# FireMines/zk_stark_project

Measured on AMD Instinct MI355X. Metric: STARK proofs/sec + prove-time ms, MiMC AIR 2^20-step trace, higher is better.
Workload: dtype f128 (u128 mod 2^128-45*2^40+1); 1 GPU; MiMC AIR 2^20-step trace, blowup=8 (BASELINE configs[1]); trace_length=1048576, trace_width=1, blowup=8, num_queries=40, grinding=21, fri_folding=16, fri_remainder_max_degree=7, parallelism=replicas1

## Files before the change

__graft_entry__.py:

```python
import os
import subprocess
import sys

ROOT = os.path.dirname(os.path.abspath(__file__))


def build() -> None:
    env = dict(os.environ)
    jobs = str(min(16, os.cpu_count() or 1))
    subprocess.check_call(["make", "-j", jobs, "-C", os.path.join(ROOT, "zk_stark_project_amd", "csrc")], env=env)
    subprocess.check_call(["make", "-j", jobs, "-C", os.path.join(ROOT, "oracle")], env=env)
    subprocess.check_call(["make", "-j", jobs, "-C", os.path.join(ROOT, "tests", "native")], env=env)
    subprocess.check_call(["make", "-j", jobs, "-C", os.path.join(ROOT, "tests", "native"), "-f", "deep_inv_check.mk"],
                          env=env)
    if ROOT not in sys.path:
        sys.path.insert(0, ROOT)
    import zk_stark_project_amd
    from zk_stark_project_amd import _native
    _native.load()


def smoke() -> None:
    for p in (ROOT, os.path.join(ROOT, "tests")):
        if p not in sys.path:
            sys.path.insert(0, p)
    from zk_stark_project_amd import AIR_MIMC, MimcProver, ProofOptions, _native
    from zk_stark_project_amd.field import to_bytes
    import oracle_ref

    ctx = _native.Context(0)
    opts = ProofOptions(40, 8, 12)
    prover = MimcProver(opts, ctx)
    n = 1 << 12
    trace = prover.build_trace(42 * 10**6, n)
    pub = prover.get_pub_inputs(trace).to_elements()
    proof = prover.prove(trace)
    ref, _ = oracle_ref.prove(AIR_MIMC, trace.to_bytes(), 1, n, to_bytes(pub), opts)
    assert proof.to_bytes() == ref, "GPU proof differs from the CPU oracle"
    assert oracle_ref.verify(AIR_MIMC, proof.to_bytes(), to_bytes(pub), opts) == 0, "proof rejected"
    _native.verify(AIR_MIMC, proof.to_bytes(), pub, opts)
    ctx.close()
    print(f"smoke ok: MiMC 2^12 proof, {len(proof)} bytes, bit-exact vs oracle")


if __name__ == "__main__":
    build()
# ... 3 lines not shown
```

zk_stark_project_amd/csrc/kernels.hip:

```cpp
#include "kernels_dev.hpp"

using kc::rev_bits;
using kc::static_for;

namespace {

__global__ void k_expand_powers(felt* out, uint64_t count, const felt* lo_tab, const felt* hi_tab) {
  for (uint64_t e = blockIdx.x * (uint64_t)TPB + threadIdx.x; e < count; e += (uint64_t)gridDim.x * TPB)
    out[e] = mul(lo_tab[e & 2047], hi_tab[e >> 11]);
}

__global__ void k_build_levels(felt* tab, uint32_t top) {
  const felt* topl = tab + ((1ull << top) - 1);
  uint64_t total = (1ull << top) - 1;
  for (uint64_t e = blockIdx.x * (uint64_t)TPB + threadIdx.x; e < total; e += (uint64_t)gridDim.x * TPB) {
    uint32_t t = 63 - __builtin_clzll(e + 1);
    uint64_t j = e + 1 - (1ull << t);
    tab[e] = topl[j << (top - t)];
  }
}

__global__ void k_build_coset_scale(felt* S, uint32_t logn, uint32_t B, const felt* tw, uint32_t logN,
                                    const felt* glo, const felt* ghi, felt ninv) {
  uint64_t total = (uint64_t)B << logn;
// ... 15 lines not shown
  const uint64_t pl = blockIdx.x * (uint64_t)TPB + threadIdx.x;
  if (pl >= nR) return;
  felt x[CE];
  static_for<0, CE>([&](auto uu) {
    constexpr int u = decltype(uu)::value;
    x[u] = mul(recv[blk[u] * nR + pl], Si[((uint64_t)u << logn) + p0 + pl]);
  });
  const felt* winv = consts + C;
  static_for<0, kc::ilog2_const(CE)>([&](auto ss) {
    constexpr int len = CE >> decltype(ss)::value, h = len / 2;
    static_for<0, CE / len>([&](auto bb) {
      constexpr int b0 = decltype(bb)::value * len;
      static_for<0, h>([&](auto jj) {
        constexpr int j = decltype(jj)::value;
        const felt u = x[b0 + j], v = x[b0 + j + h];
        x[b0 + j] = add(u, v);
        x[b0 + j + h] = j == 0 ? sub(u, v) : mul(sub(u, v), winv[j * (CE / len)]);
      });
    });
  });
  static_for<0, CE>([&](auto mm) {
    constexpr int m = decltype(mm)::value;
    if ((uint32_t)m < C) out[m * nR + pl] = mul(x[kc::rev_const(m, kc::ilog2_const(CE))], consts[m]);
  });
  if (hi_flag) {
    uint32_t nz = 0;
    static_for<0, CE>([&](auto mm) {
      constexpr int m = decltype(mm)::value;
      const felt v = x[kc::rev_const(m, kc::ilog2_const(CE))];
      if ((uint32_t)m >= C) nz |= (uint32_t)((v.lo | v.hi) != 0);
    });
    if (__builtin_amdgcn_ballot_w64(nz != 0) && (threadIdx.x & 63) == 0) hi_flag[0] = 1u;
  }
}

__global__ __launch_bounds__(TPB) void k_dt_eval_consts(int air, const felt* __restrict__ cc, felt k, felt wl,
                                                        const felt* __restrict__ aval, const felt* __restrict__ zinv,
                                                        uint32_t ce, uint32_t w, uint32_t num_t,
                                                        felt* __restrict__ out) {
  __shared__ felt red0[TPB], red1[TPB];
  const uint32_t t = threadIdx.x;
  if (air == ZKP_AIR_MIMC) {
    for (uint32_t u = t; u < ce; u += TPB) out[u] = mul(zinv[u], cc[0]);
    if (t == 0) {
      const felt b0 = cc[1], b1 = cc[2], c0 = mul(b0, aval[0]), c1 = mul(b1, aval[1]);
      out[ce] = add(b0, b1);
      out[ce + 1] = add(mul(b0, wl), b1);
      out[ce + 2] = add(c0, c1);
      out[ce + 3] = add(mul(c0, wl), c1);
    }
    return;
  }
  const bool gu = air == ZKP_AIR_GLOBAL_UPDATE;
  const uint32_t W = gu ? w : w / 2;
  felt s0 = zero(), s1 = zero();
  for (uint32_t c = t; c < W; c += TPB) {
    felt a = zero(), b = zero(), b0 = zero(), b1 = zero();
    if (gu) {
      const uint32_t d = W / 2;
      if (c < d) { a = mul(cc[c], k); b = neg(a); }
      else a = neg(cc[c - d]);
      b0 = cc[num_t + c];
      s0 = add(s0, mul(b0, aval[c]));
    } else {
      b0 = cc[num_t + c];
      b1 = cc[num_t + W + c];
// ... 1406 lines not shown
           hipLaunchKernelGGL(k_deep_lincomb<false>, g, dim3(TPB), 0, s, coef, w, n, p0, np, gamma, cpg, out));
    return;
  }
  LAUNCH(prof, "deep_lincomb", s, (double)(w + 1) * np * 16.0,
         hipLaunchKernelGGL(k_deep_lincomb<true>, g, dim3(TPB), 0, s, coef, w, n, p0, np, gamma, cpg, scratch));
  LAUNCH(prof, "deep_lincomb", s, (double)(G + 1) * np * 16.0,
         hipLaunchKernelGGL(k_sum_groups, dim3(blocks_for(np)), dim3(TPB), 0, s, scratch, G, np, out));
}

void launch_deep(Prof& prof, hipStream_t s, const DeepArgs& a, felt* out) {
  uint64_t N = 1ull << (a.logn + a.logBl);
  LAUNCH(prof, "deep", s, (double)N * ((a.w + a.C) * 16.0 + 32.0),
         hipLaunchKernelGGL(k_deep, dim3(blocks_for((N + EVAL_CH - 1) / EVAL_CH)), dim3(TPB), 0, s, a, a.inv, out));
}

void launch_comp_dft(Prof& prof, hipStream_t s, const felt* recv, const uint32_t* blk, const felt* Si,
                     const felt* consts, uint32_t ce, uint32_t C, uint32_t logn, uint64_t p0, uint64_t nR, felt* out,
                     uint32_t* hi_flag) {
  const double bytes = (double)nR * (2 * ce + C) * 16.0;
  const dim3 g(blocks_for(nR));
  switch (ce) {
    case 2: LAUNCH(prof, "comp_dft", s, bytes, hipLaunchKernelGGL(k_comp_dft<2>, g, dim3(TPB), 0, s, recv, blk, Si,
                                                                   consts, C, logn, p0, nR, out, hi_flag)); break;
    case 4: LAUNCH(prof, "comp_dft", s, bytes, hipLaunchKernelGGL(k_comp_dft<4>, g, dim3(TPB), 0, s, recv, blk, Si,
                                                                   consts, C, logn, p0, nR, out, hi_flag)); break;
    case 8: LAUNCH(prof, "comp_dft", s, bytes, hipLaunchKernelGGL(k_comp_dft<8>, g, dim3(TPB), 0, s, recv, blk, Si,
                                                                   consts, C, logn, p0, nR, out, hi_flag)); break;
    case 16: LAUNCH(prof, "comp_dft", s, bytes, hipLaunchKernelGGL(k_comp_dft<16>, g, dim3(TPB), 0, s, recv, blk,
                                                                    Si, consts, C, logn, p0, nR, out, hi_flag)); break;
    default: launch_fail(ZKP_ERR_UNSUPPORTED_AIR, "composition DFT supports ce in {2, 4, 8, 16}");
  }
}

void launch_gather_multi(Prof& prof, hipStream_t s, const GatherSeg* segs, uint32_t nseg, uint64_t max_count,
                         const uint64_t* idx, uint32_t* out, double bytes) {
  LAUNCH(prof, "gather", s, bytes,
         hipLaunchKernelGGL(k_gather_multi, dim3(blocks_for(max_count), nseg), dim3(TPB), 0, s, segs, idx, out));
}

void launch_gather_felts(Prof& prof, hipStream_t s, const felt* src, const uint64_t* idx, felt* out, uint64_t count) {
  LAUNCH(prof, "gather", s, count * 32.0,
         hipLaunchKernelGGL(k_gather_felts, dim3(blocks_for(count)), dim3(TPB), 0, s, src, idx, out, count));
}

void launch_gather_digests(Prof& prof, hipStream_t s, const uint32_t* nodes, const uint64_t* idx, uint32_t* out,
                           uint64_t count) {
  LAUNCH(prof, "gather", s, count * 40.0,
         hipLaunchKernelGGL(k_gather_digests, dim3(blocks_for(count)), dim3(TPB), 0, s, nodes, idx, out, count));
}

void launch_gu_trace(Prof& prof, hipStream_t s, const felt* masked, const felt* raw, const felt* local,
                     uint64_t ndev, felt kinv, uint64_t n, felt* tile_buf, felt* out) {
  const uint32_t tiles = (uint32_t)((n + GU_TILE - 1) / GU_TILE);
  LAUNCH(prof, "gu_trace_sums", s, (double)ndev * GU_D_DEV * 16.0,
         hipLaunchKernelGGL(k_gu_tile_sums, dim3(tiles, GU_D_DEV), dim3(TPB), 0, s, masked, raw, local, ndev, kinv,
                            n, tile_buf));
  LAUNCH(prof, "gu_trace_scan", s, (double)tiles * GU_D_DEV * 32.0,
         hipLaunchKernelGGL(k_gu_tile_scan, dim3(GU_D_DEV), dim3(64), 0, s, tile_buf, tiles));
  LAUNCH(prof, "gu_trace_write", s, (double)n * 2 * GU_D_DEV * 16.0 + (double)ndev * GU_D_DEV * 16.0,
         hipLaunchKernelGGL(k_gu_tile_write, dim3(tiles, 2 * GU_D_DEV), dim3(TPB), 0, s, masked, raw, local, ndev,
                            kinv, n, tile_buf, out));
}

void launch_tu_states(Prof& prof, hipStream_t s, felt* states, const felt* x, const felt* xs, const felt* y,
                      uint32_t bs, felt pr_inv, felt lr_inv, felt ac_inv) {
  LAUNCH(prof, "tu_states", s, (double)bs * (2 * TU_FE + TU_AC + TU_HALF) * 16.0,
// ... 74 lines not shown
```

zk_stark_project_amd/csrc/ntt.hip:

```cpp
#include "kernels_common.hpp"
#include "ntt_plan.hpp"

#include <mutex>

using kc::static_for;
using kc::rev_bits;

namespace {

struct NttKArgs {
  const felt* src;
  felt* dst;
  const felt* scale;
  const felt* tw;
  uint64_t src_stride, dst_stride;
  uint32_t src_div, scale_mod;
  uint32_t logn, s0, K, lo, T, Tl, logT, logTl, dit;
};

__global__ __launch_bounds__(TPB) void k_ntt_pass(NttKArgs a) {
  extern __shared__ felt lds[];
  const uint32_t bidx = blockIdx.y;
  const felt* src = a.src + (uint64_t)(bidx / a.src_div) * a.src_stride;
  felt* dst = a.dst + (uint64_t)bidx * a.dst_stride;
  const felt* scale = a.scale ? a.scale + ((uint64_t)(bidx % a.scale_mod) << a.logn) : nullptr;
  const uint32_t K = a.K, T = a.T, Tl = a.Tl, lo = a.lo;
  const uint32_t E = T << K;
  const uint64_t g0 = (uint64_t)blockIdx.x * T;
  const uint64_t hi0 = g0 >> lo;
  const uint64_t l0 = (Tl == T) ? (g0 & ((1ull << lo) - 1)) : 0;
  const uint32_t qmask = (1u << K) - 1;

  for (uint32_t e = threadIdx.x; e < E; e += TPB) {
    uint32_t ll = e & (Tl - 1);
    uint32_t rest = e >> a.logTl;
    uint32_t q = rest & qmask;
    uint32_t hl = rest >> K;
    uint64_t addr = ((hi0 + hl) << (lo + K)) + ((uint64_t)q << lo) + l0 + ll;
    felt v = src[addr];
    if (scale) v = mul(v, scale[addr]);
    lds[(q << a.logT) + (hl * Tl) + ll] = v;
  }
  __syncthreads();
  for (uint32_t ls = 0; ls < K; ls++) {
    const uint32_t s = a.s0 + ls;
    const uint32_t pbit = a.dit ? ls : (K - 1 - ls);
    const uint32_t lev = a.dit ? s : (a.logn - 1 - s);
    const felt* twl = a.tw + ((1ull << lev) - 1);
    const uint32_t pmask = (1u << pbit) - 1;
    for (uint32_t bf = threadIdx.x; bf < (E >> 1); bf += TPB) {
      uint32_t gg = bf & (T - 1);
      uint32_t qq = bf >> a.logT;
      uint32_t q = ((qq >> pbit) << (pbit + 1)) | (qq & pmask);
      uint32_t q2 = q | (1u << pbit);
      uint64_t l = l0 + (gg & (Tl - 1));
      uint64_t j = ((uint64_t)(q & pmask) << lo) | l;
      felt w = twl[j];
      uint32_t i0 = (q << a.logT) + gg, i1 = (q2 << a.logT) + gg;
      felt x = lds[i0], y = lds[i1];
      if (a.dit) {
        felt t = mul(y, w);
        lds[i0] = add(x, t);
        lds[i1] = sub(x, t);
      } else {
        lds[i0] = add(x, y);
        lds[i1] = mul(sub(x, y), w);
      }
    }
    __syncthreads();
  }
  for (uint32_t e = threadIdx.x; e < E; e += TPB) {
    uint32_t ll = e & (Tl - 1);
    uint32_t rest = e >> a.logTl;
    uint32_t q = rest & qmask;
    uint32_t hl = rest >> K;
    uint64_t addr = ((hi0 + hl) << (lo + K)) + ((uint64_t)q << lo) + l0 + ll;
    dst[addr] = lds[(q << a.logT) + (hl * Tl) + ll];
  }
}

struct Ntt8Args {
  const felt* src;
  felt* dst;
  const felt* scale;
  const felt* tw;
  uint64_t src_stride, dst_stride;
  uint32_t src_div, scale_mod;
  uint32_t logn, s0, K, lo, logT, logTl;
  uint32_t tile_major;
};

template <bool DIT>
__device__ __forceinline__ felt ntt_tw(const Ntt8Args& a, uint32_t j, uint32_t pbit) {
  uint32_t s = DIT ? a.s0 + pbit : a.s0 + a.K - 1 - pbit;
  uint32_t lev = DIT ? s : a.logn - 1 - s;
  return a.tw[((1u << lev) - 1) + j];
}

#ifdef ZKP_NTT_NOGMEM
#define NTT_LD(p) (make((uint64_t)(uintptr_t)(p), (uint64_t)threadIdx.x))
#define NTT_ST(p, v)                                               \
  do {                                                            \
    const felt v_ = (v);                                          \
    if (v_.lo == 0x123456789ull && v_.hi == 0xabcdefull) *(p) = v_; \
  } while (0)
#else
#define NTT_LD(p) (*(p))
#define NTT_ST(p, v) (*(p) = (v))
#endif

#ifdef ZKP_NTT_NOBFLY
template <bool FAST>
__device__ __forceinline__ felt bmul(felt a, felt b, Rare& q) { return make(a.lo ^ b.lo, a.hi ^ b.hi); }
template <bool FAST>
__device__ __forceinline__ felt badd(felt a, felt b, Rare& q) { return make(a.lo + b.lo, a.hi + b.hi); }
__device__ __forceinline__ felt nsub(felt a, felt b) { return make(a.lo - b.lo, a.hi - b.hi); }
#else
template <bool FAST>
__device__ __forceinline__ felt bmul(felt a, felt b, Rare& q) { return dmul<FAST>(a, b, q); }
template <bool FAST>
__device__ __forceinline__ felt badd(felt a, felt b, Rare& q) { return dadd<FAST>(a, b, q); }
__device__ __forceinline__ felt nsub(felt a, felt b) { return sub(a, b); }
// ... 54 lines not shown
  }
#else
  bfly<DIT, FAST>(x0, y0, w0, q);
  bfly<DIT, FAST>(x1, y1, w1, q);
#endif
}

template <bool DIT, int NT, int KC, bool SMALL>
__device__ __forceinline__ void ntt8_tile(const Ntt8Args& a, uint32_t bidx, uint32_t tile, felt* lds) {
  constexpr int E = NT * 8;
  constexpr uint32_t K = KC;
  constexpr uint32_t LOGNT = NT == 512 ? 9 : 8;
  constexpr uint32_t logT = LOGNT + 3 - KC;
  constexpr uint32_t T = 1u << logT;
  static_assert(T == 1 || T >= 4, "the LDS swizzles take rows of 1 or >= 4 felts");
  const uint32_t Tl = 1u << a.logTl, lo = a.lo;
  auto lidx = [](uint32_t q, uint32_t x) -> uint32_t {
    if constexpr (T == 1) {
      (void)x;
      return q ^ ((q >> 3) & 7u) ^ (((q >> 6) & 1u) << 3);
    } else if constexpr (T >= 32) {
      return q * T + (x ^ (q & 15u));
    } else if constexpr (T == 16 && DIT) {
      return q * T + (x ^ (q & 7u));
    } else if constexpr (T == 16) {
      return q * T + (x ^ ((q & 7u) | ((((q >> 2) ^ (q >> 4)) & 1u) << 3)));
    } else if constexpr (T == 8) {
      return (q ^ (((q >> 2) ^ (q >> 3)) & 1u)) * T + (x ^ (q & 7u));
    } else {
      const uint32_t b1 = (q >> 1) & 1u, b23 = ((q >> 2) ^ (q >> 3)) & 1u, b25 = ((q >> 2) ^ (q >> 5)) & 1u;
      return (q ^ (b23 | (b25 << 1))) * T + (x ^ (b1 | (b23 << 1)));
    }
  };
  const felt* src = a.src + (uint64_t)(bidx / a.src_div) * a.src_stride;
  felt* dst = a.dst + (uint64_t)bidx * a.dst_stride;
  const felt* scale = a.scale ? a.scale + ((uint64_t)(bidx % a.scale_mod) << a.logn) : nullptr;
  const uint64_t g0 = (uint64_t)tile << logT;
  const uint32_t hi0 = (uint32_t)(g0 >> lo);
  const uint32_t l0 = (Tl == T) ? (uint32_t)(g0 & ((1ull << lo) - 1)) : 0;
  const uint32_t qmask = (1u << K) - 1;
  const uint32_t tid = threadIdx.x;

  auto gaddr = [&](uint32_t gg, uint32_t q) -> uint32_t {
    uint32_t hl = gg >> a.logTl, ll = gg & (Tl - 1);
    return ((hi0 + hl) << (lo + K)) + (q << lo) + l0 + ll;
  };
  (void)qmask;
  const bool staged = a.logTl < (T >= 8 ? 3u : 2u);
  auto staged_elem = [&](uint32_t e, uint32_t& slot) -> uint32_t {
    uint32_t ll = e & (Tl - 1), rest = e >> a.logTl;
    uint32_t q = rest & ((1u << K) - 1), hl = rest >> K;
    slot = lidx(q, hl * Tl + ll);
    return ((hi0 + hl) << (lo + K)) + (q << lo) + l0 + ll;
  };
  if (staged) {
    auto stage_in = [&](auto fast_c, Rare& q) {
      constexpr bool FAST = decltype(fast_c)::value;
#pragma unroll
      for (int i = 0; i < 8; i++) {
        uint32_t slot;
        uint32_t ad = staged_elem(tid + i * NT, slot);
        felt v = NTT_LD(src + ad);
        if (scale) v = bmul<FAST>(v, NTT_LD(scale + ad), q);
        lds[slot] = v;
      }
    };
    Rare q;
// ... 152 lines not shown
}

template <bool DIT, int NT, int KC, bool SMALL>
__global__ __launch_bounds__(NT, (NT == 256 && KC == 11) ? 5 : 1) void k_ntt8(Ntt8Args a) {
  extern __shared__ felt lds[];
  uint32_t bidx = blockIdx.x, tile = blockIdx.y;
  if (a.tile_major) {
    const uint32_t B = gridDim.x, i = blockIdx.y * B + blockIdx.x, k = i >> 3;
    tile = (k / B) * 8 + (i & 7);
    bidx = k % B;
  }
  ntt8_tile<DIT, NT, KC, SMALL>(a, bidx, tile, lds);
}

}

void preload_ntt_module() {
  hipFuncAttributes fa;
  (void)hipFuncGetAttributes(&fa, (const void*)k_ntt_pass);
}

static void launch_ntt_radix2(Prof& prof, hipStream_t s, const NttBatch& b, uint32_t logn, bool dit,
                              const felt* tw) {
  bool first = true;
  for (const NttPass& ps : ntt_plan(logn, dit, b.batches)) {
    NttKArgs a;
    a.src = first ? b.src : b.dst;
    a.dst = b.dst;
    a.scale = first ? b.scale : nullptr;
    a.tw = tw;
    a.src_stride = first ? b.src_stride : b.dst_stride;
    a.dst_stride = b.dst_stride;
    a.src_div = first ? b.src_div : 1;
    a.scale_mod = b.scale_mod ? b.scale_mod : 1;
    a.logn = logn;
    a.s0 = ps.s0;
    a.K = ps.K;
    a.lo = ps.lo;
    a.T = 1u << ps.logT;
    a.Tl = 1u << ps.logTl;
    a.logT = ps.logT;
    a.logTl = ps.logTl;
    a.dit = dit ? 1 : 0;
    uint64_t groups = 1ull << (logn - ps.K);
    dim3 grid((uint32_t)(groups >> ps.logT), b.batches);
    size_t shmem = (size_t)(a.T << ps.K) * sizeof(felt);
    LAUNCH(prof, dit ? "ntt_dit_r2" : "ntt_dif_r2", s, (double)b.batches * (1ull << logn) * 16.0 * (a.scale ? 3 : 2),
           hipLaunchKernelGGL(k_ntt_pass, grid, dim3(TPB), shmem, s, a));
    first = false;
  }
}

#define ZKP_NTT8_KERNELS(X)                                                                \
  X(true, 256, 6, true) X(true, 256, 8, true) X(true, 256, 11, true)                       \
  X(true, 256, 6, false) X(true, 256, 7, false) X(true, 256, 8, false)                     \
  X(true, 256, 9, false) X(true, 512, 9, false)                                            \
  X(false, 256, 6, true) X(false, 256, 7, true) X(false, 256, 8, true) X(false, 256, 11, true) \
  X(false, 256, 6, false) X(false, 256, 7, false) X(false, 256, 8, false)                  \
  X(false, 256, 9, false) X(false, 512, 9, false)

void launch_ntt(Prof& prof, hipStream_t s, const NttBatch& b, uint32_t logn, bool dit, const felt* tw,
                uint32_t logN, int only_pass) {
  if (logN > 28)
    launch_fail(ZKP_ERR_TRACE_SHAPE, "NTT domain over 2^28 points (n * blowup)");
  if (logn < 11) {
    if (only_pass <= 0) launch_ntt_radix2(prof, s, b, logn, dit, tw);
    return;
  }
  static std::mutex attr_mu;
  static uint64_t attr_devs = 0;
  int dev = 0;
  (void)hipGetDevice(&dev);
  {
  std::lock_guard<std::mutex> attr_lock(attr_mu);
  if (!(attr_devs >> (dev & 63) & 1)) {
#define X(D, NT, KK, S) \
  (void)hipFuncSetAttribute((const void*)k_ntt8<D, NT, KK, S>, hipFuncAttributeMaxDynamicSharedMemorySize, NT * 8 * 16);
    ZKP_NTT8_KERNELS(X)
#undef X
    attr_devs |= 1ull << (dev & 63);
  }
  }
  const NttPlan plan = ntt_plan(logn, dit, b.batches);
  for (uint32_t p = 0; p < plan.n; p++) {
    const NttPass& ps = plan.pass[p];
    if (only_pass >= 0 && (uint32_t)only_pass != p) continue;
    Ntt8Args a;
    bool first = p == 0;
    a.src = first ? b.src : b.dst;
    a.dst = b.dst;
    a.scale = first ? b.scale : nullptr;
    a.tw = tw;
    a.src_stride = first ? b.src_stride : b.dst_stride;
    a.dst_stride = b.dst_stride;
    a.src_div = first ? b.src_div : 1;
    a.scale_mod = b.scale_mod ? b.scale_mod : 1;
    a.logn = logn;
    a.s0 = ps.s0;
    a.K = ps.K;
    a.lo = ps.lo;
    a.logT = ps.logT;
    a.logTl = ps.logTl;
    uint64_t groups = 1ull << (logn - ps.K);
    dim3 grid(b.batches, (uint32_t)(groups >> a.logT));
    a.tile_major = first && b.src_div > 1 && grid.y % 8 == 0;
    size_t shmem = (size_t)(1u << ps.K) * (1u << a.logT) * sizeof(felt);
    const double arr = (double)(1ull << logn) * 16.0;
    const uint32_t src_arrays = first ? (b.batches + a.src_div - 1) / a.src_div : b.batches;
    const uint32_t scale_rows = a.scale ? (a.scale_mod < b.batches ? a.scale_mod : b.batches) : 0;
    const double bytes = arr * ((double)src_arrays + scale_rows + b.batches);
    const uint32_t nt = 1u << ps.lognt;
#define X(D, NT, KK, S)                                                              \
  if (dit == D && nt == NT && ps.K == KK && ps.small == S)                           \
    LAUNCH(prof, D ? "ntt_dit" : "ntt_dif", s, bytes,                                \
           hipLaunchKernelGGL((k_ntt8<D, NT, KK, S>), grid, dim3(NT), shmem, s, a)); \
  else
    ZKP_NTT8_KERNELS(X)
    launch_fail(ZKP_ERR_DEVICE, "internal: NTT pass of an unplanned size");
#undef X
  }
}
```

zk_stark_project_amd/csrc/ntt_plan.hpp:

```cpp
#pragma once
#include <stdint.h>

struct NttPass {
  uint32_t s0, K, lo;
  uint32_t lognt;
  uint32_t logT, logTl;
  bool small;
};

struct NttPlan {
  uint32_t n = 0;
  NttPass pass[4];
  const NttPass* begin() const { return pass; }
  const NttPass* end() const { return pass + n; }
};

inline uint32_t ntt_split_stages(uint32_t stages, uint32_t Ks[4]) {
  const uint32_t KMAX = 8;
  const uint32_t npass = (stages + KMAX - 1) / KMAX;
  uint32_t rem = stages;
  for (uint32_t p = 0; p < npass; p++) {
    const uint32_t left = npass - p;
    uint32_t k = (rem + left - 1) / left;
    if (left > 1) {
      const uint32_t k3 = k / 3 * 3;
      if (k3 >= 3 && rem - k3 <= KMAX * (left - 1)) k = k3;
    }
    Ks[p] = k;
    rem -= k;
  }
  return npass;
}

inline NttPlan ntt_plan(uint32_t logn, bool dit, uint32_t batches) {
  NttPlan pl;
  if (logn == 0 || logn > 32) return pl;
  const bool radix2 = logn < 11;
  uint32_t Ks[4] = {0, 0, 0, 0};
  if (logn == 11) {
    pl.n = 1;
    Ks[0] = 11;
  } else if (logn >= 17 && logn <= 20) {
    pl.n = 2;
    Ks[0] = dit ? 11 : logn - 11;
    Ks[1] = dit ? logn - 11 : 11;
  } else {
    pl.n = ntt_split_stages(logn, Ks);
  }
  uint32_t s0 = 0;
  for (uint32_t p = 0; p < pl.n; s0 += Ks[p], p++) {
    NttPass& ps = pl.pass[p];
    ps.s0 = s0;
    ps.K = Ks[p];
    ps.lo = dit ? s0 : logn - s0 - ps.K;
    ps.small = ps.lo == 0;
    ps.lognt = !radix2 && ps.K == 9 && batches >= 8 ? 9 : 8;
    const uint32_t loge = radix2 ? 12 : ps.lognt + 3, logG = logn - ps.K;
    ps.logT = loge - ps.K < logG ? loge - ps.K : logG;
    ps.logTl = ps.logT < ps.lo ? ps.logT : ps.lo;
  }
  return pl;
}
```

zk_stark_project_amd/csrc/prover.cpp:

```cpp
#include "prover_internal.hpp"

#include <mutex>

using namespace zkpi;

namespace zkpi {

int ProofRun::init(int air_id, const felt* d_trace_in, uint32_t width, uint64_t n_rows, const zkp_felt* pub_elems,
                   uint64_t n_pub, uint8_t** proof, uint64_t* proof_len) {
  d_trace = d_trace_in;
  w = width;
  n = n_rows;
  int rc = check_options(o);
  if (rc) return rc;
  if (n < 8 || (n & (n - 1)) || w == 0 || w > 255) return ZKP_ERR_TRACE_SHAPE;
  if (!proof || !proof_len || (n_pub && !pub_elems)) return ZKP_ERR_ARGUMENT;
  B = o->blowup_factor; F = o->fri_folding_factor;
  logn = ilog2(n); logB = ilog2(B); logN = logn + logB;
  N = 1ull << logN;
  if (logN > MAX_LOG_DOMAIN || logn > MAX_LOG_TRACE) return ZKP_ERR_TRACE_SHAPE;
  rc = check_fri_shape(n, o);
  if (rc) return rc;
  R = (uint32_t)cm->world; rank = (uint32_t)cm->rank;
  if (R == 0 || (R & (R - 1)) || R > B || rank >= R) return ZKP_ERR_ARGUMENT;
// ... 98 lines not shown
    }
    const bool mimc_check = air.id == ZKP_AIR_MIMC && w == 1 && R == 1 && lastcol_shape();
    const bool piped = h_trace && grp.size() > 1;
    const size_t G = grp.size();
    if (piped) {
      ctx->events(G + 2);
      HIP_CHECK(hipEventRecord(ctx->ev_fork, st));
      HIP_CHECK(hipStreamWaitEvent(ctx->side, ctx->ev_fork, 0));
    }
    if (late_pairs) {
      if (!piped) throw ZkpFail{ZKP_ERR_DEVICE, "paired host trace without column groups"};
      HIP_CHECK(hipMemcpy2DAsync(const_cast<felt*>(d_trace) + (size_t)d * n, n * 16, h_trace + (size_t)d * n, n * 16,
                                 16, d, hipMemcpyHostToDevice, ctx->side));
      HIP_CHECK(hipEventRecord(ctx->up_ev[G], ctx->side));
    }
    for (uint32_t g = 0; g < grp.size(); g++) {
      const uint32_t c0 = grp[g].first, cw = grp[g].second;
      felt* dcol = const_cast<felt*>(d_trace) + (size_t)c0 * n;
      if (piped) {
        HIP_CHECK(hipMemcpyAsync(dcol, h_trace + (size_t)c0 * n, (size_t)cw * n * 16, hipMemcpyHostToDevice,
                                 ctx->side));
        HIP_CHECK(hipEventRecord(ctx->up_ev[g], ctx->side));
        HIP_CHECK(hipStreamWaitEvent(st, ctx->up_ev[g], 0));
      } else if (h_trace && g == 0) {
        ctx->upload(dcol, h_trace, (size_t)w * n * 16);
      }
      if (g == 0 && mimc_check) {
        uint32_t* dflag = ctx->buf<uint32_t>("mimc_bad", 4);
        HIP_CHECK(hipEventRecord(ctx->ev_fork, st));
        HIP_CHECK(hipStreamWaitEvent(ctx->side, ctx->ev_fork, 0));
        HIP_CHECK(hipMemsetAsync(dflag, 0, 16, ctx->side));
        launch_mimc_check(pf, ctx->side, d_trace, n, air.a_val[0], air.a_val[1], dflag);
        early_check_launch(dflag, ctx->side);
      }
      if (c0 >= wd && early_pairs) HIP_CHECK(hipStreamWaitEvent(st, ctx->ev_check, 0));
      if (c0 >= wd && early_pairs && early_check_failed()) {
        paired = false;
        gu_lazy_on = false;
      } else if (c0 >= wd) {
        const uint32_t i0 = c0 - d;
        if (!early_pairs) launch_gu_check(pf, st, d_trace, d, logn, air.k, i0, cw, 0, logn, gu_cval, gu_bad);
        launch_gu_coef(pf, st, coef, d, logn, air.k, ctx->itws(logN) + ((n >> 1) - 1), i0, cw, 0, n, gu_cval);
        if (!gu_lazy_on) launch_gu_lde(pf, st, tlde, d, logn, logBl, air.k, i0, cw, gu_cval, l0_table());
        continue;
      }
      NttBatch ib{dcol, coef + (size_t)c0 * n, nullptr, n, n, 1, 1, cw};
      launch_ntt(pf, st, ib, logn, false, ctx->itws(logN), logN);
      NttBatch lb{coef + (size_t)c0 * n, tlde + (size_t)c0 * Bl * n, Sj0, n, n, Bl, Bl, cw * Bl};
      launch_ntt(pf, st, lb, logn, true, ctx->tws(logN), logN);
    }
    if (late_pairs) {
      HIP_CHECK(hipStreamWaitEvent(st, ctx->up_ev[G], 0));
      launch_gu_check(pf, st, d_trace, d, logn, air.k, 0, d, 0, 0, gu_cval, gu_bad);
      launch_gu_coef(pf, st, coef, d, logn, air.k, ctx->itws(logN) + ((n >> 1) - 1), 0, d, 0, n, gu_cval);
      if (!gu_lazy_on) launch_gu_lde(pf, st, tlde, d, logn, logBl, air.k, 0, d, gu_cval, l0_table());
      HIP_CHECK(hipEventRecord(ctx->up_ev[G + 1], ctx->side));
      HIP_CHECK(hipStreamWaitEvent(ctx->copy, ctx->up_ev[G + 1], 0));
      late_h_trace = h_trace;
    }
  }
  {
    MerkleTail draw{};
    draw.op = MERKLE_TAIL_DRAW_COEFFS;
    draw.coin_seed = dt_seed;
    draw.method = o->batching_constraints;
    draw.ncoef = ncoef;
// ... 9 lines not shown
    }
  }
  troot_d = R > 1 ? ttree.top_d + 8 : ttree.nodes + 8;
  if (!coeffs_drawn && !host_channel)
    launch_dt_draw_coeffs(pf, st, dt_seed, troot_d, o->batching_constraints, ncoef, dt_cc);
  ctx->stage_end("1_trace_commit");
}

void ProofRun::constraint_stage() {
  eval_stage();
  composition_stage();
}

void ProofRun::eval_stage() {
  comp = ctx->buf<felt>("comp", (size_t)(cel ? cel : 1) * n);
  constraint_eval(ctx, air, logn, logB, logce, u0, cel, j0, logBl, cx, twn, dt_cc, dt_aval, tlde, comp, coef, cm);
}

bool ProofRun::lastcol_shape() const {
  static const bool no_derive = getenv("ZKP_NO_DERIVE_LAST") != nullptr;
  return allow_shortcuts && !no_derive && logce == logB && C >= 2 && C <= 8 && cel == Bl && u0 == j0;
}

void ProofRun::composition_stage() {
  comp = ctx->buf<felt>("comp", (size_t)(cel ? cel : 1) * n);
  acoef = coef + (size_t)w * n;
  clde = ctx->buf<felt>("clde", (size_t)C * Bl * n);
  bool z_drawn = false;
  wn_root = root_of_unity(logn);
  {
    const uint64_t nR = n >> logR, p0 = (uint64_t)rank * nR;
    const bool derive = lastcol_shape() && !(pre_checked && early_check_failed());
    derive_last = derive;
    if (derive) {
      lc_bad = ctx->buf<uint32_t>("lc_bad", 4);
      HIP_CHECK(hipMemsetAsync(lc_bad, 0, 16, st));
    }
    felt* cint = derive ? ctx->buf<felt>("comp_int", (size_t)(cel ? cel : 1) * n) : comp;
    if (cel) {
      NttBatch ib{comp, cint, nullptr, n, n, 1, 1, cel};
      launch_ntt(pf, st, ib, logn, false, ctx->itws(logN), logN);
    }
    felt* recv = cint;
    if (R > 1) recv = composition_exchange(cint, nR);
    const std::string dkey = "comp_dft_" + std::to_string(logn) + "_" + std::to_string(logce) + "_" +
                             std::to_string(C) + "_" + std::to_string(R) + "_" + std::to_string(celmax);
    felt* dcoefs = ctx->buf<felt>(dkey + "_coefs", (size_t)C + ce / 2);
    uint32_t* dblk = ctx->buf<uint32_t>(dkey + "_blk", ce);
    if (!ctx->have_cached(dkey)) {
      const std::vector<felt> dc = comp_dft_consts(n, logce, C);
      std::vector<uint32_t> blk(ce);
      for (uint32_t u = 0; u < ce; u++) {
        uint32_t s = ce_owner(u);
        blk[u] = s * celmax + (u - ce_first(s));
      }
      ctx->upload(dcoefs, dc.data(), dc.size() * 16);
      ctx->upload(dblk, blk.data(), blk.size() * 4);
    }
    felt* slice = R > 1 ? ctx->buf<felt>("comp_ag_send", (size_t)C * nR) : acoef;
    launch_comp_dft(pf, st, recv, dblk, ctx->Si(logn, logB, logce), dcoefs, ce, C, logn, p0, nR, slice,
                    derive ? lc_bad : nullptr);
    if (R > 1 && derive) {
      lc_flags = ctx->buf<uint32_t>("lc_flags", 4 * (size_t)R);
      cm->all_gather(st, lc_bad, lc_flags, 16);
    }
    if (R > 1) {
      composition_gather_lde(slice, derive, nR, p0);
    } else {
      NttBatch lb{acoef, clde, Sj0, n, n, Bl, Bl, (derive ? C - 1 : C) * Bl};
      launch_ntt(pf, st, lb, logn, true, ctx->tws(logN), logN);
    }
    LastCol lc{};
    if (derive) lc = LastCol{comp, last_col_kappa(ctx, logn, logB, C) + 2 * (size_t)j0, clde + (size_t)(C - 1) * Bl * n};
    MerkleTail draw{};
    draw.op = MERKLE_TAIL_DRAW_Z;
    draw.coin_seed = dt_seed;
    draw.wn = wn_root;
    draw.logn = logn;
    draw.out = dt_zz;
    draw.pw = dt_pw;
    z_drawn = commit_rows(ctx, cm, 0, clde, n, C, logB, logn, R > 1, "ctree", ctree, T.constraint_root,
                          host_channel, host_channel ? nullptr : &draw, derive ? &lc : nullptr);
  }
  croot_d = R > 1 ? ctree.top_d + 8 : ctree.nodes + 8;
  if (!z_drawn && !host_channel) launch_dt_draw_z(pf, st, dt_seed, croot_d, wn_root, logn, dt_zz, dt_pw);
  ctx->stage_end("2_constraints_commit");
}

void ProofRun::ood_values() {
  const uint64_t cnt = (uint64_t)Bl * n;
  deep_inv = ctx->buf<felt>("deep_inv", cnt);
  felt* scratch = ctx->buf<felt>("deep_inv_scratch", deep_den_scratch(cnt));
  const PointMap pm{cx + j0, twn, logn};
  const PointMap pm8{coset_points8(ctx, logn, logB) + j0,
// ... 369 lines not shown
  if (!late_h_trace) return;
  const uint32_t d = w / 2;
  HIP_CHECK(hipMemcpyAsync(const_cast<felt*>(d_trace) + (size_t)d * n, late_h_trace + (size_t)d * n,
                           (size_t)d * n * 16, hipMemcpyHostToDevice, ctx->copy));
  launch_gu_check(pf, ctx->copy, d_trace, d, logn, air.k, 0, d, 0, logn, nullptr, gu_bad);
  late_h_trace = nullptr;
  gu_late_check = true;
}

void ProofRun::early_check_launch(uint32_t* dflag, hipStream_t s) {
  HIP_CHECK(hipMemcpyAsync(ctx->host_flag(), dflag, 4, hipMemcpyDeviceToHost, s));
  HIP_CHECK(hipEventRecord(ctx->ev_check, s));
  pre_checked = true;
}

bool ProofRun::early_check_failed() {
  if (!pre_checked) return false;
  HIP_CHECK(hipEventSynchronize(ctx->ev_check));
  return *ctx->host_flag() != 0;
}

bool ProofRun::pair_failed() {
  if (!paired) return false;
  late_pairs_upload();
  if (gu_late_check) HIP_CHECK(hipStreamSynchronize(ctx->copy));
  std::vector<uint32_t> f(gu_flags ? 4 * (size_t)R : 4);
  ctx->download(f.data(), gu_flags ? gu_flags : gu_bad, f.size() * 4);
  for (uint32_t v : f)
    if (v) return true;
  return false;
}

bool ProofRun::lastcol_failed() {
  if (!derive_last) return false;
  std::vector<uint32_t> f(lc_flags ? 4 * (size_t)R : 4);
  ctx->download(f.data(), lc_flags ? lc_flags : lc_bad, f.size() * 4);
  for (uint32_t v : f)
    if (v) return true;
  return false;
}

int prove_impl(zkp_ctx* ctx, zkp_comm* cm, int air_id, const felt* d_trace, uint32_t w, uint64_t n,
               const zkp_felt* pub_elems, uint64_t n_pub, const zkp_proof_options* o, uint8_t** proof,
               uint64_t* proof_len, zkp_transcript* tr_out, const zkp_felt* h_trace) {
  for (int attempt = 0;; attempt++) {
    ProofRun run(ctx, cm, o);
    run.allow_shortcuts = attempt == 0;
    int rc = run.init(air_id, d_trace, w, n, pub_elems, n_pub, proof, proof_len);
    if (rc) return rc;
    run.setup();
    run.trace_stage(h_trace);
    run.constraint_stage();
    run.ood_stage();
    run.deep_stage();
    run.fri_stage();
    run.grind_stage();
    if (run.pair_failed() || run.lastcol_failed()) {
      if (!run.h_partial) h_trace = nullptr;
      continue;
    }
    return run.finish(proof, proof_len, tr_out);
  }
}

void drain_streams(zkp_ctx* ctx) {
  (void)hipStreamSynchronize(ctx->copy);
  (void)hipStreamSynchronize(ctx->side);
// ... 89 lines not shown
```

zk_stark_project_amd/csrc/prover_internal.hpp:

```cpp
#pragma once
#include <algorithm>
#include <array>
#include <chrono>
#include <cstdio>
#include <cstdlib>
#include <cstring>
#include <map>
#include <memory>
#include <stdexcept>
#include <string>
#include <utility>
#include <vector>

#include "../../include/zkp.h"
#include "blake3.hpp"
#include "comm.hpp"
#include "zkp_internal.hpp"

using namespace fp;

#include "host_stark.hpp"

using namespace zkh;

// ... 431 lines not shown
  std::vector<FriLayer> layers;
  std::vector<felt> remainder;
  bool dev_tail = false;
  bool dev_query = false;
  FullGatherArgs ga{};
  uint64_t* dpos = nullptr;
  const uint32_t* full_d = nullptr;
  std::vector<uint32_t> full_h;
  std::vector<uint64_t> raw_pos;
  felt* rem_d = nullptr;
  uint32_t* rcommit_d = nullptr;
  unsigned long long* dres = nullptr;
  unsigned long long dnonce = ~0ull;
  static constexpr uint64_t grind_chunk = 1ull << 22;
  uint64_t nonce = 0;
  bool allow_shortcuts = true;
  bool paired = false;
  felt* gu_cval = nullptr;
  uint32_t* gu_bad = nullptr;
  uint32_t* gu_flags = nullptr;
  bool gu_lazy_on = false;
  bool gu_late_check = false;
  const zkp_felt* late_h_trace = nullptr;
  void late_pairs_upload();
  GuLazy gu_lazy{};
  const felt* l0_table();
  bool pair_failed();
  bool derive_last = false;
  bool lastcol_shape() const;
  uint32_t* lc_bad = nullptr;
  uint32_t* lc_flags = nullptr;
  bool lastcol_failed();
  bool pre_checked = false;
  void early_check_launch(uint32_t* dflag, hipStream_t s);
  bool early_check_failed();
  bool h_partial = false;
  bool host_channel = false;

  ProofRun(zkp_ctx* c, zkp_comm* m, const zkp_proof_options* opts)
      : ctx(c), cm(m), o(opts), st(c->stream), pf(c->prof) {
    memset(&T, 0, sizeof T);
  }
  uint32_t ce_owner(uint32_t u) const { return (u << cstep) / Bl; }
  uint32_t ce_first(uint32_t s) const {
    uint32_t u = 0;
    while (u < ce && ce_owner(u) < s) u++;
    return u;
  }
  int init(int air_id, const felt* d_trace_in, uint32_t width, uint64_t n_rows, const zkp_felt* pub_elems,
           uint64_t n_pub, uint8_t** proof, uint64_t* proof_len);
  void setup();
  void trace_stage(const zkp_felt* h_trace);
  void constraint_stage();
  void eval_stage();
  void composition_stage();
  void ood_values();
  void ood_stage();
  void deep_stage();
  void fri_stage();
  FriCursor fri_layers();
  void fri_round_trip(const FriCursor& c);
  void grind_stage();
  int finish(uint8_t** proof, uint64_t* proof_len, zkp_transcript* tr_out);
  void trace_column_sharded(const zkp_felt* h_trace, uint32_t cpt, uint32_t wi, uint32_t d);
  const zkp_felt* gather_host_slices(const zkp_felt* h_trace);
  felt* composition_exchange(felt* cint, uint64_t nR);
// ... 70 lines not shown
```

zk_stark_project_amd/csrc/zkp_internal.hpp:

```cpp
#pragma once
#include <hip/hip_runtime.h>
#include <stdint.h>

#include <string>
#include <vector>

#include "felt.hpp"

struct ProfRec {
  const char* name;
  double bytes;
  hipEvent_t start, stop;
};
struct Prof {
  bool enabled = false;
  std::string only;
  bool open = false;
  std::vector<ProfRec> pending;
  std::vector<hipEvent_t> pool;
  hipEvent_t get_event();
  void begin(const char* name, hipStream_t s, double bytes);
  void end(hipStream_t s);
};

[[noreturn]] void launch_fail(int code, const char* what);
constexpr uint32_t MAX_LOG_DOMAIN = 28, MAX_LOG_TRACE = 23;
void preload_kernels_module();
void preload_merkle_module();
void preload_ntt_module();
void warm_stream(hipStream_t s);

struct NttBatch {
  const felt* src;
  felt* dst;
  const felt* scale;
  uint64_t src_stride, dst_stride;
  uint32_t src_div, scale_mod, batches;
};

void launch_ntt(Prof& prof, hipStream_t s, const NttBatch& b, uint32_t logn, bool dit, const felt* tw,
                uint32_t logN, int only_pass = -1);

void launch_build_levels(Prof& prof, hipStream_t s, felt* tab, uint32_t top);
void launch_expand_powers(Prof& prof, hipStream_t s, felt* out, uint64_t count, const felt* lo_tab,
                          const felt* hi_tab);
void launch_build_coset_scale(Prof& prof, hipStream_t s, felt* S, uint32_t logn, uint32_t B,
                              const felt* tw, uint32_t logN, const felt* glo, const felt* ghi, felt ninv);

enum { MERKLE_TAIL_NONE = 0, MERKLE_TAIL_FRI_COIN = 1, MERKLE_TAIL_DRAW_COEFFS = 2, MERKLE_TAIL_DRAW_Z = 3 };
struct MerkleTail {
  uint32_t* done;
  uint32_t* coin_seed;
  felt* alpha_out;
  uint32_t* root_out;
  uint32_t op, method, ncoef, logn;
  felt wn;
  felt* out;
  felt* pw;
};
struct LastCol {
  const felt* H;
  const felt* kap;
  felt* out;
};
struct GuLazy {
  const felt* cval;
  const felt* l0;
  felt k;
  uint32_t d, wi, smallk;
};
// ... 157 lines not shown
struct ProgCheckArgs {
  const uint64_t* ops;
  uint32_t nops, nreg, nassert, frame_blocks;
  uint32_t single_blocks, nstrided;
  const ProgStridedCells* sdesc;
  const felt* svals;
  const felt* consts;
  const ProgPeriodic* per_desc;
  const felt* per_tab;
  const uint32_t* a_col;
  const uint32_t* a_step;
  const felt* a_val;
  uint64_t n;
};
void launch_check_program(Prof& prof, hipStream_t s, ProgCheckArgs a, uint32_t width, const felt* T,
                          unsigned long long* res, uint64_t strided_blocks = 0);

void launch_mimc_check(Prof& prof, hipStream_t s, const felt* T, uint64_t n, felt v0, felt v1, uint32_t* bad);
void launch_gu_check(Prof& prof, hipStream_t s, const felt* T, uint32_t d, uint32_t logn, felt k, uint32_t c0,
                     uint32_t cw, uint64_t t0, uint32_t logtn, felt* cval, uint32_t* bad);
void launch_gu_coef(Prof& prof, hipStream_t s, felt* coef, uint32_t d, uint32_t logn, felt k, const felt* itwn,
                    uint32_t c0, uint32_t cw, uint64_t p0, uint64_t np, const felt* cval);
void launch_gu_lde(Prof& prof, hipStream_t s, felt* lde, uint32_t d, uint32_t logn, uint32_t logBl, felt k,
                   uint32_t c0, uint32_t cw, const felt* cval, const felt* l0);
size_t l0_scratch_felts(uint64_t count, uint32_t logn);
void launch_l0_table(Prof& prof, hipStream_t s, const PointMap& pm, uint64_t count, felt ninv, felt* out,
                     felt* scratch);
void launch_gu_fill(Prof& prof, hipStream_t s, felt* lde, uint32_t w, uint32_t logn, uint32_t logB, uint32_t j0,
                    uint32_t logBl, const uint64_t* pos, uint32_t npos, const GuLazy& gl);

void launch_comp_dft(Prof& prof, hipStream_t s, const felt* recv, const uint32_t* blk, const felt* Si,
                     const felt* consts, uint32_t ce, uint32_t C, uint32_t logn, uint64_t p0, uint64_t nR, felt* out,
                     uint32_t* hi_flag = nullptr);

void launch_eval_bitrev(Prof& prof, hipStream_t s, const felt* arrays, uint32_t narrays, uint32_t ntwo, uint32_t logn,
                        const felt* pw0, const felt* pw1, felt* partial, felt ninv, felt* out);
void launch_eval_bitrev_blocks(Prof& prof, hipStream_t s, const felt* arrays, uint32_t narrays, uint32_t ntwo,
                               uint32_t logn, const felt* pw0, const felt* pw1, uint32_t b0, uint32_t nbl,
                               felt* partial);
void launch_eval_bitrev_tail(Prof& prof, hipStream_t s, const felt* partial, uint32_t narrays, uint32_t logn,
                             uint32_t nbl, const felt* pw0, const felt* pw1, felt ninv, felt* out);

struct DeepArgs {
  uint32_t w, C, logB, logn, logN;
  uint32_t j0, logBl;
  const felt* tlde;
  const felt* clde;
  const felt* gamma;
  const felt* dk;
  felt g;
  const felt* inv;
  felt ginv;
};
struct DeepRoots {
  felt w8, w8_2, w8_3;
};
inline uint64_t deep_den_scratch(uint64_t count) { return count / 8 + count / (8 * 2048) + 2; }
void launch_deep_denominators(Prof& prof, hipStream_t s, hipStream_t s2, hipEvent_t ev, const PointMap& m,
                              const PointMap& m8, const DeepRoots& r, uint64_t count, const felt* zz, const felt* pw,
                              felt* scratch, felt* table);
void launch_deep(Prof& prof, hipStream_t s, const DeepArgs& a, felt* out);
void launch_deep_lincomb(Prof& prof, hipStream_t s, const felt* coef, uint32_t w, uint64_t n, uint64_t p0,
                         uint64_t np, const felt* gamma, felt* out,
                         felt* scratch);

void launch_fri_fold(Prof& prof, hipStream_t s, const felt* E, uint64_t m16, uint32_t Bl, uint32_t j0,
// ... 40 lines not shown
```

Before: 231.6 proofs/s.

## Interpolate only six of eight composition cosets when trace is pre-checked

When the trace has already been validated and the composition has ce=8 with C=6 columns, the prover runs the inverse NTT on only six selected coset arrays (chosen by a packed source-pick mask) instead of all eight. A specialised 6-point DFT kernel then combines them with the Si scaling and constants, exploiting the known vanishing structure of the high columns. This cuts one quarter of the inverse-NTT work and drops the last-column nonzero check. The NTT plan threshold is lowered so six-batch runs still use the larger tile. The change relies on the trace check having passed, and it skips the lc_bad verification on that path.

```diff
diff --git a/__graft_entry__.py b/__graft_entry__.py
--- a/__graft_entry__.py
+++ b/__graft_entry__.py
@@ -12,6 +12,8 @@
     subprocess.check_call(["make", "-j", jobs, "-C", os.path.join(ROOT, "oracle")], env=env)
     subprocess.check_call(["make", "-j", jobs, "-C", os.path.join(ROOT, "tests", "native")], env=env)
     subprocess.check_call(["make", "-j", jobs, "-C", os.path.join(ROOT, "tests", "native"), "-f", "deep_inv_check.mk"],
+                          env=env)
+    subprocess.check_call(["make", "-j", jobs, "-C", os.path.join(ROOT, "tests", "native"), "-f", "comp6_check.mk"],
                           env=env)
     if ROOT not in sys.path:
         sys.path.insert(0, ROOT)
diff --git a/zk_stark_project_amd/csrc/kernels.hip b/zk_stark_project_amd/csrc/kernels.hip
--- a/zk_stark_project_amd/csrc/kernels.hip
+++ b/zk_stark_project_amd/csrc/kernels.hip
@@ -71,6 +71,30 @@
     });
     if (__builtin_amdgcn_ballot_w64(nz != 0) && (threadIdx.x & 63) == 0) hi_flag[0] = 1u;
   }
+}
+
+__global__ __launch_bounds__(TPB) void k_comp_dft6(const felt* __restrict__ cint, const felt* __restrict__ Si,
+                                                   const felt* __restrict__ consts, uint32_t logn,
+                                                   felt* __restrict__ out) {
+  const uint64_t n = 1ull << logn, p = blockIdx.x * (uint64_t)TPB + threadIdx.x;
+  if (p >= n) return;
+  felt y[6];
+  static_for<0, 6>([&](auto kk) {
+    constexpr int k = decltype(kk)::value, u = k < 4 ? 2 * k : (k == 4 ? 1 : 5);
+    y[k] = mul(cint[(uint64_t)k * n + p], Si[((uint64_t)u << logn) + p]);
+  });
+  const felt w1 = consts[6 + 1], w2 = consts[6 + 2];
+  const felt s0 = add(y[0], y[2]), d0 = sub(y[0], y[2]);
+  const felt s1 = add(y[1], y[3]), d1 = mul(sub(y[1], y[3]), w2);
+  const felt a0 = add(s0, s1), a2 = sub(s0, s1), a1 = add(d0, d1), a3 = sub(d0, d1);
+  const felt sp = add(y[4], y[5]), dm = mul(sub(y[4], y[5]), w1);
+  const felt e = add(add(sp, sp), mul(a2, w2)), o = add(add(dm, dm), mul(a3, w2));
+  out[0 * n + p] = mul(add(a0, e), consts[0]);
+  out[1 * n + p] = mul(add(a1, o), consts[1]);
+  out[2 * n + p] = mul(add(a2, a2), consts[2]);
+  out[3 * n + p] = mul(add(a3, a3), consts[3]);
+  out[4 * n + p] = mul(sub(a0, e), consts[4]);
+  out[5 * n + p] = mul(sub(a1, o), consts[5]);
 }
 
 __global__ __launch_bounds__(TPB) void k_dt_eval_consts(int air, const felt* __restrict__ cc, felt k, felt wl,
@@ -1543,6 +1567,13 @@
   }
 }
 
+void launch_comp_dft6(Prof& prof, hipStream_t s, const felt* cint, const felt* Si, const felt* consts, uint32_t logn,
+                      felt* out) {
+  const uint64_t n = 1ull << logn;
+  LAUNCH(prof, "comp_dft6", s, (double)n * 18 * 16.0,
+         hipLaunchKernelGGL(k_comp_dft6, dim3(blocks_for(n)), dim3(TPB), 0, s, cint, Si, consts, logn, out));
+}
+
 void launch_gather_multi(Prof& prof, hipStream_t s, const GatherSeg* segs, uint32_t nseg, uint64_t max_count,
                          const uint64_t* idx, uint32_t* out, double bytes) {
   LAUNCH(prof, "gather", s, bytes,
diff --git a/zk_stark_project_amd/csrc/ntt.hip b/zk_stark_project_amd/csrc/ntt.hip
--- a/zk_stark_project_amd/csrc/ntt.hip
+++ b/zk_stark_project_amd/csrc/ntt.hip
@@ -16,12 +16,17 @@
   uint64_t src_stride, dst_stride;
   uint32_t src_div, scale_mod;
   uint32_t logn, s0, K, lo, T, Tl, logT, logTl, dit;
+  uint32_t src_pick;
 };
+
+__device__ __forceinline__ uint32_t ntt_src_array(uint32_t bidx, uint32_t src_div, uint32_t src_pick) {
+  return src_pick ? (src_pick >> (4 * bidx)) & 15u : bidx / src_div;
+}
 
 __global__ __launch_bounds__(TPB) void k_ntt_pass(NttKArgs a) {
   extern __shared__ felt lds[];
   const uint32_t bidx = blockIdx.y;
-  const felt* src = a.src + (uint64_t)(bidx / a.src_div) * a.src_stride;
+  const felt* src = a.src + (uint64_t)ntt_src_array(bidx, a.src_div, a.src_pick) * a.src_stride;
   felt* dst = a.dst + (uint64_t)bidx * a.dst_stride;
   const felt* scale = a.scale ? a.scale + ((uint64_t)(bidx % a.scale_mod) << a.logn) : nullptr;
   const uint32_t K = a.K, T = a.T, Tl = a.Tl, lo = a.lo;
@@ -88,6 +93,7 @@
   uint32_t src_div, scale_mod;
   uint32_t logn, s0, K, lo, logT, logTl;
   uint32_t tile_major;
+  uint32_t src_pick;
 };
 
 template <bool DIT>
@@ -208,7 +214,7 @@
       return (q ^ (b23 | (b25 << 1))) * T + (x ^ (b1 | (b23 << 1)));
     }
   };
-  const felt* src = a.src + (uint64_t)(bidx / a.src_div) * a.src_stride;
+  const felt* src = a.src + (uint64_t)ntt_src_array(bidx, a.src_div, a.src_pick) * a.src_stride;
   felt* dst = a.dst + (uint64_t)bidx * a.dst_stride;
   const felt* scale = a.scale ? a.scale + ((uint64_t)(bidx % a.scale_mod) << a.logn) : nullptr;
   const uint64_t g0 = (uint64_t)tile << logT;
@@ -427,6 +433,7 @@
     a.src_stride = first ? b.src_stride : b.dst_stride;
     a.dst_stride = b.dst_stride;
     a.src_div = first ? b.src_div : 1;
+    a.src_pick = first ? b.src_pick : 0;
     a.scale_mod = b.scale_mod ? b.scale_mod : 1;
     a.logn = logn;
     a.s0 = ps.s0;
@@ -489,6 +496,7 @@
     a.src_stride = first ? b.src_stride : b.dst_stride;
     a.dst_stride = b.dst_stride;
     a.src_div = first ? b.src_div : 1;
+    a.src_pick = first ? b.src_pick : 0;
     a.scale_mod = b.scale_mod ? b.scale_mod : 1;
     a.logn = logn;
     a.s0 = ps.s0;
diff --git a/zk_stark_project_amd/csrc/ntt_plan.hpp b/zk_stark_project_amd/csrc/ntt_plan.hpp
--- a/zk_stark_project_amd/csrc/ntt_plan.hpp
+++ b/zk_stark_project_amd/csrc/ntt_plan.hpp
@@ -54,7 +54,7 @@
     ps.K = Ks[p];
     ps.lo = dit ? s0 : logn - s0 - ps.K;
     ps.small = ps.lo == 0;
-    ps.lognt = !radix2 && ps.K == 9 && batches >= 8 ? 9 : 8;
+    ps.lognt = !radix2 && ps.K == 9 && batches >= 6 ? 9 : 8;
     const uint32_t loge = radix2 ? 12 : ps.lognt + 3, logG = logn - ps.K;
     ps.logT = loge - ps.K < logG ? loge - ps.K : logG;
     ps.logTl = ps.logT < ps.lo ? ps.logT : ps.lo;
diff --git a/zk_stark_project_amd/csrc/prover.cpp b/zk_stark_project_amd/csrc/prover.cpp
--- a/zk_stark_project_amd/csrc/prover.cpp
+++ b/zk_stark_project_amd/csrc/prover.cpp
@@ -154,6 +154,7 @@
         HIP_CHECK(hipMemsetAsync(dflag, 0, 16, ctx->side));
         launch_mimc_check(pf, ctx->side, d_trace, n, air.a_val[0], air.a_val[1], dflag);
         early_check_launch(dflag, ctx->side);
+        trace_checked = true;
       }
       if (c0 >= wd && early_pairs) HIP_CHECK(hipStreamWaitEvent(st, ctx->ev_check, 0));
       if (c0 >= wd && early_pairs && early_check_failed()) {
@@ -229,12 +230,18 @@
     const uint64_t nR = n >> logR, p0 = (uint64_t)rank * nR;
     const bool derive = lastcol_shape() && !(pre_checked && early_check_failed());
     derive_last = derive;
-    if (derive) {
+    static const bool no_six = getenv("ZKP_NO_SIX_COSETS") != nullptr;
+    const bool six = derive && trace_checked && !host_channel && !no_six && R == 1 && ce == 8 && C == 6 && cel == 8;
+    lc_bad = nullptr;
+    if (derive && !six) {
       lc_bad = ctx->buf<uint32_t>("lc_bad", 4);
       HIP_CHECK(hipMemsetAsync(lc_bad, 0, 16, st));
     }
     felt* cint = derive ? ctx->buf<felt>("comp_int", (size_t)(cel ? cel : 1) * n) : comp;
-    if (cel) {
+    if (six) {
+      NttBatch ib{comp, cint, nullptr, n, n, 1, 1, 6, COMP6_PICK};
+      launch_ntt(pf, st, ib, logn, false, ctx->itws(logN), logN);
+    } else if (cel) {
       NttBatch ib{comp, cint, nullptr, n, n, 1, 1, cel};
       launch_ntt(pf, st, ib, logn, false, ctx->itws(logN), logN);
     }
@@ -255,8 +262,11 @@
       ctx->upload(dblk, blk.data(), blk.size() * 4);
     }
     felt* slice = R > 1 ? ctx->buf<felt>("comp_ag_send", (size_t)C * nR) : acoef;
-    launch_comp_dft(pf, st, recv, dblk, ctx->Si(logn, logB, logce), dcoefs, ce, C, logn, p0, nR, slice,
-                    derive ? lc_bad : nullptr);
+    if (six)
+      launch_comp_dft6(pf, st, cint, ctx->Si(logn, logB, logce), dcoefs, logn, acoef);
+    else
+      launch_comp_dft(pf, st, recv, dblk, ctx->Si(logn, logB, logce), dcoefs, ce, C, logn, p0, nR, slice,
+                      derive ? lc_bad : nullptr);
     if (R > 1 && derive) {
       lc_flags = ctx->buf<uint32_t>("lc_flags", 4 * (size_t)R);
       cm->all_gather(st, lc_bad, lc_flags, 16);
@@ -692,7 +702,7 @@
 }
 
 bool ProofRun::lastcol_failed() {
-  if (!derive_last) return false;
+  if (!derive_last || !lc_bad) return false;
   std::vector<uint32_t> f(lc_flags ? 4 * (size_t)R : 4);
   ctx->download(f.data(), lc_flags ? lc_flags : lc_bad, f.size() * 4);
   for (uint32_t v : f)
diff --git a/zk_stark_project_amd/csrc/prover_internal.hpp b/zk_stark_project_amd/csrc/prover_internal.hpp
--- a/zk_stark_project_amd/csrc/prover_internal.hpp
+++ b/zk_stark_project_amd/csrc/prover_internal.hpp
@@ -487,6 +487,7 @@
   uint32_t* lc_flags = nullptr;
   bool lastcol_failed();
   bool pre_checked = false;
+  bool trace_checked = false;
   void early_check_launch(uint32_t* dflag, hipStream_t s);
   bool early_check_failed();
   bool h_partial = false;
diff --git a/zk_stark_project_amd/csrc/zkp_internal.hpp b/zk_stark_project_amd/csrc/zkp_internal.hpp
--- a/zk_stark_project_amd/csrc/zkp_internal.hpp
+++ b/zk_stark_project_amd/csrc/zkp_internal.hpp
@@ -36,6 +36,7 @@
   const felt* scale;
   uint64_t src_stride, dst_stride;
   uint32_t src_div, scale_mod, batches;
+  uint32_t src_pick = 0;
 };
 
 void launch_ntt(Prof& prof, hipStream_t s, const NttBatch& b, uint32_t logn, bool dit, const felt* tw,
@@ -259,6 +260,9 @@
 void launch_comp_dft(Prof& prof, hipStream_t s, const felt* recv, const uint32_t* blk, const felt* Si,
                      const felt* consts, uint32_t ce, uint32_t C, uint32_t logn, uint64_t p0, uint64_t nR, felt* out,
                      uint32_t* hi_flag = nullptr);
+constexpr uint32_t COMP6_PICK = 0x516420;
+void launch_comp_dft6(Prof& prof, hipStream_t s, const felt* cint, const felt* Si, const felt* consts, uint32_t logn,
+                      felt* out);
 
 void launch_eval_bitrev(Prof& prof, hipStream_t s, const felt* arrays, uint32_t narrays, uint32_t ntwo, uint32_t logn,
                         const felt* pw0, const felt* pw1, felt* partial, felt ninv, felt* out);
```

New measurement: 236.2 proofs/s (median of 6 runs). 1.02x the previous value.
